# DaehwanKimLab/centrifuge

Measured on NVIDIA H100. Metric: reads/sec (100 bp SE classification), higher is better.
Workload: dtype u64

## Files before the change

### centrifuge_b200/csrc/cfb200.cu

```cuda
#include "../../include/cfb200.h"
#include "cf_index.h"
#include "cf_kernels.cuh"
#include <cub/cub.cuh>

#include <algorithm>
#include <atomic>
#include <mutex>
#include <thread>
#include <fcntl.h>
#include <unistd.h>
#include <cstdarg>
#include <cstdio>
#include <cstring>
#include <set>
#include <string>
#include <vector>

using namespace cfb;

enum { M_DONE = 0, M_FTAB = 1, M_LF = 2, M_NEED = 3, M_FTABK = 4, M_TASK = 5 };

struct SearchArgs {
	IndexView v; Params p; BatchView b;
	HitRec* hits; uint32_t* nhits; uint32_t cap;
// ... 31 lines not shown
	const int mate = (int)(rem >> 1), strand = (int)(rem & 1);
	const uint32_t len = mate ? a.b.len[1][unit] : a.b.len[0][unit];
	uint64_t w = 0; uint32_t n = 0;
	if(k * 32 < len) {
		const uint64_t off = mate ? a.b.off[1][unit] : a.b.off[0][unit];
		const uint32_t cnt = min(32u, len - k * 32);
		const uint64_t lo = strand ? off + k * 32 : off + (len - k * 32 - cnt);
		#pragma unroll
		for(uint32_t g = 0; g < 32; g += 4) {
			if(g < cnt) {
				const uint32_t keep = cnt - g >= 4 ? 0xffffffffu : ((1u << (8 * (cnt - g))) - 1u);
				const uint32_t v = load4(a.b.bases, lo + g) & keep;
				const uint32_t nb = __vcmpne4(v & 0xFCFCFCFCu, 0u) & 0x01010101u;
				uint32_t b2 = v & 0x03030303u;
				if(strand) b2 ^= 0x03030303u & keep;
				b2 &= ~(nb * 3u);
				w |= (uint64_t)squeeze4x2(b2) << (2 * g);
				n |= squeeze4x1(nb) << g;
			}
		}
		if(!strand) {
			uint64_t x = __brevll(w);
			x = ((x >> 1) & 0x5555555555555555ull) | ((x & 0x5555555555555555ull) << 1);
			w = x >> (2 * (32 - cnt)); n = __brev(n) >> (32 - cnt);
		}
	}
	a.pk[i] = w; a.nm[i] = n;
}

struct WarpPool { unsigned long long base = 0, end = 0, next = 0; bool ahead = false; };
__device__ __forceinline__ void pool_ahead(WarpPool& P, unsigned long long* ctr, unsigned chunk) {
	if(!P.ahead && P.end - P.base < 32) { if((threadIdx.x & 31) == 0) P.next = atomicAdd(ctr, (unsigned long long)chunk); P.ahead = true; }
}
__device__ __forceinline__ bool pool_take(WarpPool& P, bool want, unsigned long long* ctr, unsigned long long total, unsigned chunk, unsigned long long& out) {
	const unsigned need = __ballot_sync(0xffffffffu, want);
	if(!need) return false;
	const unsigned lane = threadIdx.x & 31;
	const unsigned cnt = __popc(need), r = __popc(need & ((1u << lane) - 1u));
	const unsigned long long avail = P.end - P.base;
	unsigned long long nb = 0;
	const bool refill = avail < cnt;
	if(refill) { if(lane == 0) nb = P.ahead ? P.next : atomicAdd(ctr, (unsigned long long)chunk); nb = __shfl_sync(0xffffffffu, nb, 0); P.ahead = false; }
	unsigned long long t, lim;
	if(r < avail) { t = P.base + r; lim = P.end; }
	else { t = nb + (r - avail); lim = nb + chunk < total ? nb + chunk : total; }
	if(refill) { P.base = nb + (cnt - avail); P.end = nb + chunk < total ? nb + chunk : total; if(P.base > P.end) P.base = P.end; }
	else P.base += cnt;
	out = t;
	return want && t < lim;
}

__device__ __forceinline__ uint64_t even_bits(uint64_t x) {
	x &= 0x5555555555555555ull;
	x = (x | (x >> 1)) & 0x3333333333333333ull;
	x = (x | (x >> 2)) & 0x0f0f0f0f0f0f0f0full;
	x = (x | (x >> 4)) & 0x00ff00ff00ff00ffull;
	x = (x | (x >> 8)) & 0x0000ffff0000ffffull;
	x = (x | (x >> 16)) & 0x00000000ffffffffull;
	return x;
}

__global__ void k_build_rank16(const uint64_t* sides, uint64_t num_sides, uint64_t zside, uint32_t zoffc, uint64_t* r16) {
	const uint64_t b = (uint64_t)blockIdx.x * blockDim.x + threadIdx.x;
	if(b > num_sides * 6) return;
	const bool sentinel = b == num_sides * 6;
	const uint64_t s = sentinel ? num_sides - 1 : b / 6; const uint32_t sub = sentinel ? 6u : (uint32_t)(b - s * 6);
	const uint64_t* sd = sides + s * 16;
	uint64_t occ[4] = {sd[12], sd[13], sd[14], sd[15]};
	for(uint32_t k = 0; k < sub * 2; k++) {
		const uint64_t w = sd[k];
		const uint64_t lo = w & 0x5555555555555555ull, hi = (w >> 1) & 0x5555555555555555ull;
		const uint32_t c1 = __popcll(lo & ~hi), c2 = __popcll(hi & ~lo), c3 = __popcll(hi & lo);
		occ[1] += c1; occ[2] += c2; occ[3] += c3; occ[0] += 32 - c1 - c2 - c3;
	}
	if(s == zside && zoffc < sub * 64) occ[0] -= 1;
	for(int c = 0; c < 4; c++) {
		uint64_t bits = 0;
		if(!sentinel) {
			bits = even_bits(match2(sd[sub * 2], c)) | (even_bits(match2(sd[sub * 2 + 1], c)) << 32);
			if(c == 0 && s == zside && zoffc >= sub * 64 && zoffc < sub * 64 + 64) bits &= ~(1ull << (zoffc - sub * 64));
		}
		r16[(b * 4 + c) * 2] = occ[c]; r16[(b * 4 + c) * 2 + 1] = bits;
	}
}
__global__ void k_mark_boundaries(const uint64_t* brow, uint32_t n, uint64_t* r16) {
	const uint32_t i = blockIdx.x * blockDim.x + threadIdx.x;
	if(i < n) atomicOr((unsigned long long*)&r16[(brow[i] >> 6) * 8], 1ull << 63);
}
__global__ void k_build_ftab2(IndexView v, uint64_t n, uint64_t* ftab2) {
	const uint64_t fi = (uint64_t)blockIdx.x * blockDim.x + threadIdx.x;
	if(fi >= n) return;
	ftab2[fi * 2] = ftab_hi(v, v.ftab[fi]); ftab2[fi * 2 + 1] = ftab_lo(v, v.ftab[fi + 1]);
}
static const uint32_t kListNoLong = 0x80000000u;
static const uint32_t kListRegen = 0x40000000u;
static const uint32_t kLongLen = 22;
__host__ __device__ __forceinline__ uint32_t nh_pack(uint32_t stored, uint32_t found, bool nolong) {
	return (stored & 0x7fffu) | ((found < 0x7fffu ? found : 0x7fffu) << 15) | (nolong ? kListNoLong : 0u);
}
__host__ __device__ __forceinline__ uint32_t nh_stored(uint32_t w) { return w & 0x7fffu; }
__host__ __device__ __forceinline__ uint32_t nh_found(uint32_t w) { return (w >> 15) & 0x7fffu; }

static const uint64_t kFtabkWide = 0xFFFFFFull;
__device__ __forceinline__ uint32_t ftabk_death(uint64_t y, uint32_t e) {
	if((y >> e) & 1ull) return 0;
	if(!(y & (0x1111111111111111ull << (e & 3u)))) return 1;
	if(!(y & (0x0001000100010001ull << (e & 15u)))) return 2;
	return 3;
}
__device__ __forceinline__ void lf4(const IndexView& v, const ulonglong2* r16, uint64_t top, uint64_t bot, uint64_t t[4], uint64_t b[4]) {
	const ulonglong2* pt = r16 + r16_entry(top, 0); const ulonglong2* pb = r16 + r16_entry(bot, 0);
	#pragma unroll
	for(int c = 0; c < 4; c++) {
		const ulonglong2 et = __ldg(pt + c); const ulonglong2 eb = (pb == pt) ? et : __ldg(pb + c);
		t[c] = r16_lf(v, top, c, et.x, et.y);
		b[c] = r16_lf(v, bot, c, eb.x, eb.y);
	}
}
__global__ void __launch_bounds__(128) k_build_ftabk(IndexView v, int K, uint64_t n, bool death, ulonglong2* out) {
	const uint64_t fk = (uint64_t)blockIdx.x * blockDim.x + threadIdx.x;
	if(fk >= n) return;
	const ulonglong2* r16 = reinterpret_cast<const ulonglong2*>(v.rank16);
	const int fc = v.ftab_chars;
	const uint64_t f10 = fk & ((1ull << (2 * fc)) - 1ull);
	uint64_t top = v.ftab2[f10 * 2], bot = v.ftab2[f10 * 2 + 1];
	for(int j = fc; j < K && bot > top; j++) {
		const int c = (int)((fk >> (2 * j)) & 3);
		const ulonglong2 tq = __ldg(r16 + r16_entry(top, c)), bq = __ldg(r16 + r16_entry(bot, c));
		top = r16_lf(v, top, c, tq.x, tq.y);
		bot = r16_lf(v, bot, c, bq.x, bq.y);
	}
	if(bot <= top) { out[fk] = make_ulonglong2(0ull, ~0ull); return; }
	uint64_t y = ~0ull;
	if(death) {
		uint8_t dv[64];
		uint64_t t1[4], b1[4]; lf4(v, r16, top, bot, t1, b1);
		for(int c0 = 0; c0 < 4; c0++) {
			if(b1[c0] <= t1[c0]) { for(int r = 0; r < 16; r++) dv[c0 | (r << 2)] = 1; continue; }
			uint64_t t2[4], b2[4]; lf4(v, r16, t1[c0], b1[c0], t2, b2);
			for(int c1 = 0; c1 < 4; c1++) {
				if(b2[c1] <= t2[c1]) { for(int c2 = 0; c2 < 4; c2++) dv[c0 | (c1 << 2) | (c2 << 4)] = 2; continue; }
				uint64_t t3[4], b3[4]; lf4(v, r16, t2[c1], b2[c1], t3, b3);
				for(int c2 = 0; c2 < 4; c2++) dv[c0 | (c1 << 2) | (c2 << 4)] = b3[c2] <= t3[c2] ? 3 : 0;
			}
		}
		y = 0;
		for(int e = 0; e < 64; e++) if(dv[e] == 0) y |= 1ull << e;
		for(uint32_t e = 0; e < 64; e++) if(ftabk_death(y, e) != dv[e]) { y = ~0ull; break; }
	}
	const uint64_t w = bot - top;
	out[fk] = make_ulonglong2(top | ((w < kFtabkWide ? w : kFtabkWide) << 40), y);
}

template <int RW> struct ReadRegs {
	uint64_t rw[RW]; uint32_t nw[RW];
	__device__ __forceinline__ uint64_t word(uint32_t k) const {
		uint64_t v = 0;
		#pragma unroll
		for(int q = 0; q < RW; q++) if((uint32_t)q == k) v = rw[q];
		return v;
	}
	__device__ __forceinline__ uint32_t nword(uint32_t k) const {
		uint32_t v = 0;
		#pragma unroll
		for(int q = 0; q < RW; q++) if((uint32_t)q == k) v = nw[q];
		return v;
	}
	__device__ __forceinline__ int base(uint32_t p) const {
		const uint32_t k = p >> 5, sh = p & 31;
		return ((nword(k) >> sh) & 1u) ? 4 : (int)((word(k) >> (2 * sh)) & 3);
	}
	__device__ __forceinline__ void window(uint32_t p, uint64_t& win, uint32_t& nwin) const {
		const uint32_t k = p >> 5, sh = p & 31;
		win = shr64(word(k), 2 * sh) | shl64(word(k + 1), 64 - 2 * sh);
		nwin = (uint32_t)(((uint64_t)nword(k) | ((uint64_t)nword(k + 1) << 32)) >> sh);
	}
};

__device__ __forceinline__ void ld_if(ulonglong2& v, const void* p) {
	asm volatile("{\n\t.reg .pred p;\n\tsetp.ne.u64 p, %2, 0;\n\t@p ld.global.nc.v2.u64 {%0, %1}, [%2];\n\t}" : "+l"(v.x), "+l"(v.y) : "l"(p));
}
__device__ __forceinline__ void ld_if(uint64_t& v, const uint64_t* p, bool on) {
	asm volatile("{\n\t.reg .pred p;\n\tsetp.ne.u32 p, %2, 0;\n\t@p ld.global.nc.u64 %0, [%1];\n\t}" : "+l"(v) : "l"(p), "r"((uint32_t)on));
}
__device__ __forceinline__ void ld_if(uint32_t& v, const uint32_t* p, bool on) {
	asm volatile("{\n\t.reg .pred p;\n\tsetp.ne.u32 p, %2, 0;\n\t@p ld.global.nc.u32 %0, [%1];\n\t}" : "+r"(v) : "l"(p), "r"((uint32_t)on));
}
__device__ __forceinline__ void ld_if(uint32_t& v, const uint8_t* p, bool on) {
	asm volatile("{\n\t.reg .pred p;\n\tsetp.ne.u32 p, %2, 0;\n\t@p ld.global.nc.u8 %0, [%1];\n\t}" : "+r"(v) : "l"(p), "r"((uint32_t)on));
}

template <bool REQS, int RW>
__global__ void __launch_bounds__(kSearchThreads, !REQS && RW <= 5 ? 8 : 1) k_search_t(const SearchArgs a) {
	const ulonglong2* r16 = reinterpret_cast<const ulonglong2*>(a.v.rank16);
	const ulonglong2* ftab2 = reinterpret_cast<const ulonglong2*>(a.v.ftab2);
	const ulonglong2* ftabk = reinterpret_cast<const ulonglong2*>(a.v.ftabk);
	const uint32_t fk = a.v.ftabk ? (uint32_t)a.v.ftabk_chars : 0u;
	const uint32_t fc = (uint32_t)a.v.ftab_chars;
	const unsigned long long* w8 = reinterpret_cast<const unsigned long long*>(a.v.walk8);
	const uint32_t fd = (fk == 0 || a.p.min_hitlen < (uint32_t)a.v.ftabd_chars) ? 0u : (uint32_t)a.v.ftabd_chars;
	const uint32_t msh = a.b.n_mates == 2 ? 2u : 1u;
	ReadRegs<RW> rd;
	#pragma unroll
	for(int k = 0; k < RW; k++) { rd.rw[k] = 0; rd.nw[k] = 0; }
	uint64_t top = 0, bot = 0, fi = 0;
	uint32_t rlen = 0, tid = 0, cur = 0, dep = 0, offset = 0, nh = 0, nt = 0, slow_until = 0, fail_at = 0xffffffffu;
	bool nolong = true;
	int mode = M_NEED;
	unsigned long long q_r16 = 0, q_f2 = 0, q_fk = 0, q_w8 = 0;
	unsigned long long q_w1 = 0, q_w24 = 0, q_w5 = 0, j_row = 0, j_row_ok = 0, j_rng = 0, j_rng_ok = 0, j_w5_ok = 0;
	unsigned long long s_trips = 0, s_lreq = 0, s_cons = 0, s_rest = 0, s_task = 0, s_head = 0, s_wait = 0, s_tail = 0;
	uint32_t paths = 0; long long t_top = 0, t_issue = 0, t_data = 0;
	WarpPool pool;
	bool more = true;

	for(;;) {
		if(REQS) { paths = 0; t_top = clock64(); }
		{
			const bool want = mode == M_NEED;
			if(more) {
				unsigned long long t = 0;
				const bool got = pool_take(pool, want, a.task_ctr64, (unsigned long long)a.ntasks, a.chunk, t);
				if(want) {
					if(got) { tid = (uint32_t)t; mode = M_TASK; if(REQS) paths |= 1u << 17; }
					else mode = M_DONE;
				}
				if(__any_sync(0xffffffffu, want && !got)) more = false;
				else pool_ahead(pool, a.task_ctr64, a.chunk);
			} else if(want) mode = M_DONE;
		}
		if(!__any_sync(0xffffffffu, mode != M_DONE)) break;
		int c = 4;
		const bool lf = mode == M_LF, task = mode == M_TASK;
		bool range = false, jump = false, known_fail = false;
		const void* p0 = nullptr; const void* p1 = nullptr; uint32_t sub = 0;
		if(mode == M_FTAB) { p0 = ftab2 + fi; if(REQS) q_f2++; }
		else if(mode == M_FTABK) { p0 = ftabk + (fi & ((1ull << (2 * fk)) - 1ull)); if(REQS) q_fk++; }
		else if(lf) {
			c = rd.base(dep);
			if(c <= 3) {
				range = (bot - top) != 1;
				const uint64_t width = bot - top;
				if(dep == fail_at && !range) known_fail = true;
				else if(w8 && dep >= slow_until && rlen - dep >= 8 && bot <= a.v.walk8_rows) {
					jump = true; p0 = w8 + (top & ~1ull); sub = (uint32_t)(top & 1);
					if(range) { const uint64_t last = bot - 1; sub |= (uint32_t)(last & 1) << 1; if((last & ~1ull) != (top & ~1ull)) p1 = w8 + (last & ~1ull); }
					if(REQS) { q_w8 += p1 ? 2 : 1; if(range) j_rng++; else j_row++; }
				} else {
					p0 = r16 + r16_entry(top, c);
					if(range && (bot >> 6) != (top >> 6)) p1 = r16 + r16_entry(bot, c);
					if(REQS) { const uint32_t n = p1 ? 2 : 1; q_r16 += n; if(width == 1) q_w1 += n; else if(width <= 4) q_w24 += n; else q_w5 += n; }
				}
			}
		}
		const uint32_t unit = tid >> msh, mate = (tid >> 1) & (msh - 1u);
		const uint64_t* tpk = a.pk + (size_t)tid * a.W; const uint32_t* tnm = a.nm + (size_t)tid * a.W;
		uint32_t fl = 3;
		if(REQS) { if(p0) s_lreq++; t_issue = clock64(); }
		const bool two = p1 != nullptr;
		ulonglong2 e = make_ulonglong2(0, 0), e2 = make_ulonglong2(0, 0);
		ld_if(e, p0);
		ld_if(e2, p1);
		ld_if(rlen, (mate ? a.b.len[1] : a.b.len[0]) + unit, task);
		ld_if(fl, a.b.flags + unit, task && a.b.flags != nullptr);
		#pragma unroll
		for(int k = 0; k < RW; k++) { ld_if(rd.rw[k], tpk + k, task && (uint32_t)k < a.W); ld_if(rd.nw[k], tnm + k, task && (uint32_t)k < a.W); }
		if(REQS) {
			if(__any_sync(0xffffffffu, (e.x ^ e2.y ^ rd.rw[RW - 1] ^ rd.nw[RW - 1] ^ rlen ^ fl) == 0x9e3779b97f4a7c15ull)) s_task += 1ull << 40;
			t_data = clock64();
		}
		const ulonglong2 tq = e, bq = two ? e2 : e;
		bool ended = false, stop = false, fresh = false;
		uint64_t h_top = kOff, h_bot = kOff; uint32_t hl = 0;
		if(task) {
			if(REQS) paths |= 1u;
			#pragma unroll
			for(int k = 0; k < RW; k++) if((uint32_t)k >= a.W) { rd.rw[k] = 0; rd.nw[k] = 0; }
			nh = 0; nt = 0;
			if(!((fl >> mate) & 1) || rlen == 0) { a.nhits[tid] = 0; mode = M_NEED; }
			else { cur = 0; slow_until = 0; fail_at = 0xffffffffu; nolong = true; fresh = true; }
		} else if(mode == M_FTABK) {
			if(REQS) paths |= 2u;
			const uint32_t ext = (uint32_t)(fi >> (2 * fk));
			const uint32_t dv = ext ? ftabk_death(e.y, ext & 63u) : 0u;
			const uint64_t width = e.x >> 40;
			if(dv) {
				hl = fk + dv - 1u; h_top = h_bot = kUnk; cur += hl; ended = true;
			} else if(width != 0 && width != kFtabkWide) {
				top = e.x & kRowMask; bot = top + width; dep = cur + fk;
				if(dep < rlen) mode = M_LF; else stop = true;
			} else { fi &= (1ull << (2 * fc)) - 1ull; mode = M_FTAB; }
		} else if(mode == M_FTAB) {
			if(REQS) paths |= 4u;
			top = e.x; bot = e.y;
			dep = cur + fc;
			if(bot <= top) { hl = dep - offset; cur = dep; ended = true; }
			else if(dep < rlen) mode = M_LF;
			else stop = true;
		} else if(jump) {
			if(REQS) paths |= 8u;
			uint64_t win; uint32_t nwin; rd.window(dep, win, nwin);
			const uint64_t w = (sub & 1u) ? e.y : e.x;
			const uint64_t wl = range ? ((sub & 2u) ? bq.y : bq.x) : w;
			const uint32_t st = walk8_steps(w, win, nwin), sb = range ? walk8_steps(wl, win, nwin) : st;
			if((st & sb) == 8u) {
				if(REQS) { if(range) j_rng_ok++; else j_row_ok++; if(bot - top >= 5) j_w5_ok++; }
				top = w & kWalkRowMask; bot = (wl & kWalkRowMask) + 1; dep += 8;
				stop = dep >= rlen;
			} else {
				slow_until = dep + walk8_retry(st, sb);
				if(!range) fail_at = dep + st;
			}
		} else if(lf) {
			if(REQS) paths |= 16u;
			bool fail = c > 3 || known_fail;
			uint64_t t = 0, b = 0;
			if(!fail) {
				t = r16_lf(a.v, top, c, tq.x, tq.y);
				if(range) b = r16_lf(a.v, bot, c, bq.x, bq.y);
				else {
					if(!((tq.y >> (top & 63)) & 1ull)) fail = true;
					b = t + 1;
				}
				if(b <= t) fail = true;
			}
			if(fail) stop = true;
			else { top = t; bot = b; dep++; stop = dep >= rlen; }
		}
		if(stop) { h_top = top; h_bot = bot; hl = dep - offset; cur = dep; ended = true; }
		#pragma unroll 1
		while(ended || fresh) {
			if(ended) {
				if(REQS) paths |= 1u << 16;
				if(a.keep_short || hl >= kLongLen) {
					if(nh < a.cap) { HitRec* h = a.hits + (size_t)tid * a.cap + nh; h->top = h_top; h->bot = h_bot; h->bwoff = offset; h->len = hl; }
					else atomicExch(a.overflow, 1u);
					nh++;
				}
				nt++;
				if(hl >= a.p.min_hitlen) nolong = false;
				ended = false;
				bool done = cur >= rlen;
				if(!done) { if(hl > a.p.increment) cur += 1; if(cur + a.p.min_hitlen >= rlen) done = true; }
				if(done) { a.nhits[tid] = nh_pack(nh, nt, nolong); mode = M_NEED; break; }
			}
			if(REQS) paths |= 1u << 18;
			fresh = false;
			offset = cur; h_top = h_bot = kOff;
			if(rlen - cur < fc) { hl = rlen - cur; cur = rlen; ended = true; continue; }
			uint64_t win; uint32_t nwin; rd.window(cur, win, nwin);
			const uint32_t nbits = nwin & ((1u << fc) - 1u);
			if(nbits) { hl = (uint32_t)__ffs(nbits); cur += hl; ended = true; continue; }
			if(fk && rlen - cur >= fk && !(nwin & ((1u << fk) - 1u))) {
				fi = win & ((1ull << (2 * fk)) - 1ull);
				if(fd && rlen - cur >= fd && !(nwin & ((1u << fd) - 1u))) fi |= (64ull | ((win >> (2 * fk)) & 63ull)) << (2 * fk);
				mode = M_FTABK;
			} else {
				fi = win & ((1ull << (2 * fc)) - 1ull);
				mode = M_FTAB;
			}
		}
		if(REQS) {
			const uint32_t all = __reduce_or_sync(0xffffffffu, paths);
			s_trips++; s_cons += __popc(all & 0xffffu); s_rest += __popc(all >> 16); if(all & (1u << 17)) s_task++;
			const long long t_end = clock64(); s_head += t_issue - t_top; s_wait += t_data - t_issue; s_tail += t_end - t_data;
		}
	}
	if(REQS && a.ctr) {
		atomicAdd(&a.ctr->req_rank16, q_r16); atomicAdd(&a.ctr->req_ftab2, q_f2); atomicAdd(&a.ctr->req_ftabk, q_fk); atomicAdd(&a.ctr->req_walk8, q_w8);
		atomicAdd(&a.ctr->r16_w1, q_w1); atomicAdd(&a.ctr->r16_w2_4, q_w24); atomicAdd(&a.ctr->r16_w5, q_w5);
		atomicAdd(&a.ctr->w8_try_row, j_row); atomicAdd(&a.ctr->w8_ok_row, j_row_ok); atomicAdd(&a.ctr->w8_try_range, j_rng); atomicAdd(&a.ctr->w8_ok_range, j_rng_ok); atomicAdd(&a.ctr->w8_ok_w5, j_w5_ok);
		atomicAdd(&a.ctr->it_lane_req, s_lreq);
		if((threadIdx.x & 31) == 0) {
			atomicAdd(&a.ctr->it_warp, s_trips); atomicAdd(&a.ctr->it_consumers, s_cons); atomicAdd(&a.ctr->it_restarts, s_rest); atomicAdd(&a.ctr->it_task, s_task & ((1ull << 40) - 1ull));
			atomicAdd(&a.ctr->clk_head, s_head); atomicAdd(&a.ctr->clk_wait, s_wait); atomicAdd(&a.ctr->clk_tail, s_tail);
		}
	}
}

struct UnitArgs {
	IndexView v; Params p; BatchView b;
	HitRec* hits; uint32_t* nhits; uint32_t cap;
	uint32_t* nrows;
	uint64_t* row_off;
	unsigned long long* row_total;
	uint64_t* rows; uint32_t* ids; uint64_t rows_cap;
	Entry* entries; TaxCnt* tcs; OutRec* recs_sparse; uint32_t* nout;
	unsigned int* overflow;
	Counters* ctr;
	HitRec* regen; uint32_t* regen_n; unsigned long long* regen_ctr; uint64_t regen_slots; uint32_t full_cap; uint32_t keep_short;
};

__device__ uint32_t search_strand_dev(const IndexView& v, const Params& p, const uint8_t* fw, uint32_t len, int strand, HitRec* hits, uint32_t cap) {
	const ulonglong2* r16 = reinterpret_cast<const ulonglong2*>(v.rank16);
	const ulonglong2* ftab2 = reinterpret_cast<const ulonglong2*>(v.ftab2);
	const ulonglong2* ftabk = reinterpret_cast<const ulonglong2*>(v.ftabk);
	const uint32_t fc = (uint32_t)v.ftab_chars, fk = v.ftabk ? (uint32_t)v.ftabk_chars : 0u;
	auto base = [&](uint32_t d) -> int { return seq_at(fw, len, strand, len - 1 - d); };
	uint32_t cur = 0, n = 0;
	if(len == 0) return 0;
	for(;;) {
		HitRec h; h.bwoff = cur; uint32_t new_cur; bool done = false;
		const uint32_t offset = cur;
		if(len - cur < fc) { h.top = h.bot = kOff; h.len = len - offset; new_cur = len; done = true; }
		else {
			uint32_t firstn = 0xffffffffu; uint64_t fi = 0;
			const uint32_t span = (fk && len - cur >= fk) ? fk : fc;
			for(uint32_t i = 0; i < span; i++) { const int c = base(cur + i); if(c > 3) { firstn = i; break; } fi |= (uint64_t)c << (2 * i); }
			if(firstn < fc) { new_cur = cur + firstn + 1; h.top = h.bot = kOff; h.len = new_cur - offset; done = new_cur >= len; }
			else {
				uint64_t top = 0, bot = 0; uint32_t dep = 0; bool have = false;
				if(span == fk && fk > fc && firstn == 0xffffffffu) {
					const uint64_t x = __ldg(&ftabk[fi].x), width = x >> 40;
					if(width != 0 && width != kFtabkWide) { top = x & kRowMask; bot = top + width; dep = cur + fk; have = true; }
				}
				if(!have) { const ulonglong2 e = __ldg(ftab2 + (fi & ((1ull << (2 * fc)) - 1ull))); top = e.x; bot = e.y; dep = cur + fc; }
				if(bot <= top) { h.top = h.bot = kOff; h.len = dep - offset; new_cur = dep; done = dep >= len; }
				else {
					uint32_t slow_until = 0;
					while(dep < len) {
						const int c = base(dep);
						if(c > 3) break;
						if(v.walk8 && bot <= v.walk8_rows && len - dep >= 8 && dep >= slow_until) {
							uint64_t win = 0; uint32_t nwin = 0;
							for(uint32_t j = 0; j < 8; j++) { const int b = base(dep + j); if(b > 3) nwin |= 1u << j; else win |= (uint64_t)b << (2 * j); }
							const uint64_t et = __ldg(v.walk8 + top), eb = bot - top == 1 ? et : __ldg(v.walk8 + bot - 1);
							const uint32_t st = walk8_steps(et, win, nwin), sb = walk8_steps(eb, win, nwin);
							if((st & sb) == 8u) { top = et & kWalkRowMask; bot = (eb & kWalkRowMask) + 1; dep += 8; continue; }
							slow_until = dep + walk8_retry(st, sb);
						}
// ... 834 lines not shown
	const uint8_t* src_bases = b->bases;
	if(!pinned(b->bases)) { CK(s.h_bases.ensure(b->n_bases)); memcpy(s.h_bases.p, b->bases, b->n_bases); src_bases = s.h_bases.p; }
	CK(cudaMemcpyAsync(s.d_bases.p, src_bases, b->n_bases, cudaMemcpyHostToDevice, s.st));
	CK(s.h_off.ensure(n * nm)); CK(s.h_len.ensure(n * nm)); CK(s.h_flags.ensure(n));
	for(int m = 0; m < nm; m++) {
		const uint64_t* so = b->off[m]; const uint32_t* sl = b->len[m];
		if(!pinned(so)) { memcpy(s.h_off.p + m * n, so, n * 8); so = s.h_off.p + m * n; }
		if(!pinned(sl)) { memcpy(s.h_len.p + m * n, sl, n * 4); sl = s.h_len.p + m * n; }
		CK(cudaMemcpyAsync(s.d_off.p + m * n, so, n * 8, cudaMemcpyHostToDevice, s.st));
		CK(cudaMemcpyAsync(s.d_len.p + m * n, sl, n * 4, cudaMemcpyHostToDevice, s.st));
	}
	if(b->flags && pinned(b->flags)) CK(cudaMemcpyAsync(s.d_flags.p, b->flags, n, cudaMemcpyHostToDevice, s.st));
	else { if(b->flags) memcpy(s.h_flags.p, b->flags, n); else memset(s.h_flags.p, 3, n); CK(cudaMemcpyAsync(s.d_flags.p, s.h_flags.p, n, cudaMemcpyHostToDevice, s.st)); }
	s.bv.bases = s.d_bases.p; s.bv.flags = s.d_flags.p; s.bv.n_units = (uint32_t)n; s.bv.n_mates = nm;
	for(int m = 0; m < 2; m++) { s.bv.off[m] = m < nm ? s.d_off.p + m * n : nullptr; s.bv.len[m] = m < nm ? s.d_len.p + m * n : nullptr; }
	s.n_units = n; s.n_bases = b->n_bases; s.maxlen = maxlen;
	(void)c;
	return CFB_OK;
}

__global__ void __launch_bounds__(256) k_wlen(const uint32_t* len, uint64_t n, uint32_t* wlen) {
	const uint64_t i = (uint64_t)blockIdx.x * blockDim.x + threadIdx.x;
	if(i < n) wlen[i] = (len[i] + 31u) >> 5;
}
__global__ void __launch_bounds__(256) k_unpack(const uint64_t* __restrict__ words, const uint64_t* __restrict__ woff, uint64_t wbase, const uint32_t* __restrict__ len,
                                                uint64_t n, uint32_t W, uint8_t* bases, uint64_t* off) {
	const uint64_t t = (uint64_t)blockIdx.x * blockDim.x + threadIdx.x;
	if(t >= n * W) return;
	const uint64_t i = t / W; const uint32_t k = (uint32_t)(t - i * W);
	const uint64_t w0 = wbase + woff[i];
	if(k == 0) off[i] = w0 * 32;
	if(k * 32 >= len[i]) return;
	const uint64_t w = __ldg(words + w0 + k);
	uint32_t o[8];
	#pragma unroll
	for(int q = 0; q < 8; q++) {
		const uint32_t b = (uint32_t)(w >> (8 * q)) & 0xffu;
		o[q] = (b & 3u) | ((b & 0xcu) << 6) | ((b & 0x30u) << 12) | ((b & 0xc0u) << 18);
	}
	uint4* dst = reinterpret_cast<uint4*>(bases + (w0 + k) * 32);
	dst[0] = make_uint4(o[0], o[1], o[2], o[3]); dst[1] = make_uint4(o[4], o[5], o[6], o[7]);
}
__global__ void __launch_bounds__(256) k_set_n(const uint64_t* npos, uint64_t n, uint8_t* bases, uint64_t limit) {
	const uint64_t i = (uint64_t)blockIdx.x * blockDim.x + threadIdx.x;
	if(i < n) { const uint64_t p = npos[i]; if(p < limit) bases[p] = 4; }
}

static int stage_batch_packed(cfb_ctx* c, Slot& s, const cfb_batch_packed* b) {
	if(!b || b->n_mates < 1 || b->n_mates > 2 || !b->words || !b->len[0] || (b->n_mates == 2 && !b->len[1]) || (b->n_n && !b->n_pos))
		return fail(CFB_EINVAL, "malformed cfb_batch_packed");
	if(b->n_units >= (1ull << 30)) return fail(CFB_EINVAL, "batch too large (n_units must be < 2^30)");
	const uint64_t n = b->n_units; const int nm = b->n_mates;
	uint32_t maxlen = 0; uint64_t need_words = 0, mate_words[2] = {0, 0};
	for(int m = 0; m < nm; m++) {
		const uint32_t* L = b->len[m]; uint32_t mx = 0; uint64_t w = 0;
		for(uint64_t i = 0; i < n; i++) { const uint32_t l = L[i]; mx = l > mx ? l : mx; w += (l + 31u) >> 5; }
		maxlen = std::max(maxlen, mx); mate_words[m] = w; need_words += w;
	}
	if(need_words != b->n_words) return fail(CFB_EINVAL, "cfb_batch_packed: n_words is %llu, the lengths need %llu", (unsigned long long)b->n_words, (unsigned long long)need_words);
	if(maxlen > 60000) return fail(CFB_EINVAL, "read longer than 60000 bases");
	const uint64_t scan_blocks = (n + kScanBlock * kScanPer - 1) / (kScanBlock * kScanPer);
	CK(s.d_bases.ensure(b->n_words * 32 + 64)); CK(s.d_off.ensure(n * nm + 1)); CK(s.d_len.ensure(n * nm)); CK(s.d_flags.ensure(n));
	CK(s.d_words.ensure(b->n_words + 1)); CK(s.d_npos.ensure(b->n_n + 1)); CK(s.d_wlen.ensure(n + 1)); CK(s.d_woff.ensure(n + 2)); CK(s.bsum.ensure(scan_blocks + 1));
	auto pinned = [](const void* p) -> bool {
		cudaPointerAttributes at;
		if(cudaPointerGetAttributes(&at, p) != cudaSuccess) { cudaGetLastError(); return false; }
		return at.type == cudaMemoryTypeHost;
	};
	const uint64_t* src_words = b->words;
	if(!pinned(b->words)) { CK(s.h_words.ensure(b->n_words)); memcpy(s.h_words.p, b->words, b->n_words * 8); src_words = s.h_words.p; }
	CK(cudaMemcpyAsync(s.d_words.p, src_words, b->n_words * 8, cudaMemcpyHostToDevice, s.st));
	CK(s.h_len.ensure(n * nm)); CK(s.h_flags.ensure(n));
	for(int m = 0; m < nm; m++) {
		const uint32_t* sl = b->len[m];
		if(!pinned(sl)) { memcpy(s.h_len.p + m * n, sl, n * 4); sl = s.h_len.p + m * n; }
		CK(cudaMemcpyAsync(s.d_len.p + m * n, sl, n * 4, cudaMemcpyHostToDevice, s.st));
	}
	if(b->n_n) {
		const uint64_t* sp = b->n_pos;
		if(!pinned(sp)) { CK(s.h_off.ensure(b->n_n)); memcpy(s.h_off.p, sp, b->n_n * 8); sp = s.h_off.p; }
		CK(cudaMemcpyAsync(s.d_npos.p, sp, b->n_n * 8, cudaMemcpyHostToDevice, s.st));
	}
	if(b->flags && pinned(b->flags)) CK(cudaMemcpyAsync(s.d_flags.p, b->flags, n, cudaMemcpyHostToDevice, s.st));
	else { if(b->flags) memcpy(s.h_flags.p, b->flags, n); else memset(s.h_flags.p, 3, n); CK(cudaMemcpyAsync(s.d_flags.p, s.h_flags.p, n, cudaMemcpyHostToDevice, s.st)); }
	const uint32_t W = (maxlen + 31) / 32;
	uint64_t wbase = 0;
	CK(cudaMemsetAsync(s.scal.p + 5, 0, 8, s.st));
	for(int m = 0; m < nm && n; m++) {
		k_wlen<<<(unsigned)((n + 255) / 256), 256, 0, s.st>>>(s.d_len.p + m * n, n, s.d_wlen.p);
		k_scan_sums<<<(unsigned)scan_blocks, kScanBlock, 0, s.st>>>(s.d_wlen.p, n, s.bsum.p);
		k_scan_top<<<1, 1024, 0, s.st>>>(s.bsum.p, scan_blocks, (uint64_t*)(s.scal.p + 5));
		k_scan_apply<<<(unsigned)scan_blocks, kScanBlock, 0, s.st>>>(s.d_wlen.p, n, s.bsum.p, (const uint64_t*)(s.scal.p + 5), s.d_woff.p);
		if(W) k_unpack<<<(unsigned)((n * W + 255) / 256), 256, 0, s.st>>>(s.d_words.p, s.d_woff.p, wbase, s.d_len.p + m * n, n, W, s.d_bases.p, s.d_off.p + m * n);
		c->launches += 5;
		wbase += mate_words[m];
	}
	if(b->n_n) { k_set_n<<<(unsigned)((b->n_n + 255) / 256), 256, 0, s.st>>>(s.d_npos.p, b->n_n, s.d_bases.p, b->n_words * 32); c->launches++; }
	CK(cudaGetLastError());
	s.bv.bases = s.d_bases.p; s.bv.flags = s.d_flags.p; s.bv.n_units = (uint32_t)n; s.bv.n_mates = nm;
	for(int m = 0; m < 2; m++) { s.bv.off[m] = m < nm ? s.d_off.p + m * n : nullptr; s.bv.len[m] = m < nm ? s.d_len.p + m * n : nullptr; }
	s.n_units = n; s.n_bases = b->n_words * 32; s.maxlen = maxlen;
	return CFB_OK;
}

static int enqueue_kernels(cfb_ctx* c, Slot& s, int stage, bool time_it) {
	const uint64_t n = s.n_units; const int nm = s.bv.n_mates;
	const uint64_t ntasks = n * nm * 2;
	const uint32_t ublocks = (uint32_t)((n + 127) / 128);
	const uint64_t scan_blocks = (n + kScanBlock * kScanPer - 1) / (kScanBlock * kScanPer);
	if(n == 0) return CFB_OK;
	const SearchKernel search = search_kernel(s.maxlen, c->count);
	const bool keep_short = search == k_search_long<true> || search == k_search_long<false> || c->prm.min_hitlen < kLongLen || c->keep_short;
	if(stage == 0) {
		if(s.cap == 0) {
			s.full_cap = s.maxlen / 4 + 8;
			s.cap = keep_short ? s.full_cap : s.maxlen / kLongLen + 2;
		}
		CK(s.hits.ensure(ntasks * s.cap)); CK(s.nhits.ensure(ntasks));
		if(!keep_short) {
			s.regen_slots = std::max<uint64_t>(s.regen_slots, c->regen_slots0 ? c->regen_slots0 : std::max<uint64_t>(ntasks / 32, 1024));
			CK(s.regen.ensure(s.regen_slots * s.full_cap)); CK(s.regen_n.ensure(s.regen_slots));
			CK(cudaMemsetAsync(s.scal.p + 6, 0, sizeof(unsigned long long), s.st));
		}
		const uint32_t W = (s.maxlen + 31) / 32 + 1;
		CK(s.pk.ensure(ntasks * W + 2)); CK(s.nm.ensure(ntasks * W + 2)); CK(s.nrows.ensure(n)); CK(s.row_off.ensure(n + 1));
		CK(s.bsum.ensure(scan_blocks + 1)); CK(s.nout.ensure(n + 1)); CK(s.out_off.ensure(n + 1)); CK(s.rec_off32.ensure(n + 1));
		s.rows_cap = std::max<uint64_t>(s.rows_cap, c->rows_cap0 ? c->rows_cap0 : std::max<uint64_t>(n * 12, 4096));
	}
	CK(s.rows.ensure(s.rows_cap)); CK(s.ids.ensure(s.rows_cap)); CK(s.entries.ensure(s.rows_cap)); CK(s.tcs.ensure(s.rows_cap)); CK(s.sparse.ensure(s.rows_cap));
	s.dense_cap = s.rows_cap; CK(s.dense.ensure(s.dense_cap));
	CK(cudaMemsetAsync(s.scal.p, 0, 4 * sizeof(unsigned long long), s.st));
	if(time_it) CK(cudaEventRecord(s.ev[0], s.st));
	Counters* ctr = c->count ? c->d_ctr : nullptr;
	if(c->count && stage == 0) CK(cudaMemsetAsync(c->d_ctr, 0, sizeof(Counters), s.st));
	else if(c->count) {
		const size_t sc0 = offsetof(Counters, sc_units);
		CK(cudaMemsetAsync(reinterpret_cast<char*>(c->d_ctr) + sc0, 0, sizeof(Counters) - sc0, s.st));
	}
	UnitArgs ua; ua.v = c->view; ua.p = c->prm; ua.b = s.bv; ua.hits = s.hits.p; ua.nhits = s.nhits.p; ua.cap = s.cap;
	ua.nrows = s.nrows.p; ua.row_off = s.row_off.p; ua.row_total = s.scal.p + 3; ua.rows = s.rows.p; ua.ids = s.ids.p; ua.rows_cap = s.rows_cap;
	ua.entries = s.entries.p; ua.tcs = s.tcs.p; ua.recs_sparse = s.sparse.p; ua.nout = s.nout.p;
	ua.overflow = (unsigned int*)(s.scal.p + 2); ua.ctr = ctr;
	ua.regen = s.regen.p; ua.regen_n = s.regen_n.p; ua.regen_ctr = s.scal.p + 6; ua.regen_slots = s.regen_slots; ua.full_cap = s.full_cap; ua.keep_short = keep_short ? 1u : 0u;
	if(stage == 0) {
		SearchArgs sa; sa.v = c->view; sa.p = c->prm; sa.b = s.bv; sa.hits = s.hits.p; sa.nhits = s.nhits.p; sa.cap = s.cap;
		const uint32_t W = (s.maxlen + 31) / 32 + 1;
		sa.pk = s.pk.p; sa.nm = s.nm.p; sa.W = W; sa.keep_short = keep_short ? 1u : 0u;
		{ PackArgs pa; pa.b = s.bv; pa.pk = s.pk.p; pa.nm = s.nm.p; pa.W = W;
		  k_pack<<<(unsigned)((ntasks * W + 127) / 128), 128, 0, s.st>>>(pa); c->launches++; }
		sa.task_ctr64 = s.scal.p + 0; sa.ntasks = (uint32_t)ntasks; sa.overflow = (unsigned int*)(s.scal.p + 2); sa.ctr = ctr;
		int occ = 1;
		CK(cudaOccupancyMaxActiveBlocksPerMultiprocessor(&occ, search, kSearchThreads, 0));
		const uint64_t resident = (uint64_t)c->ix->sm_count * (uint64_t)std::max(occ, 1);
		const uint64_t warps = resident * (kSearchThreads / 32);
		sa.chunk = (uint32_t)std::min<uint64_t>(std::max<uint64_t>(ntasks / (warps * 4), 32), 256);
		const int blocks = (int)std::min<uint64_t>(resident, (ntasks + kSearchThreads - 1) / kSearchThreads);
		search<<<blocks, kSearchThreads, 0, s.st>>>(sa);
		c->launches++;
		if(time_it) CK(cudaEventRecord(s.ev[1], s.st));
		k_prep<8, false><<<ublocks, 128, 0, s.st>>>(ua); c->launches++;
	} else {
		if(time_it) CK(cudaEventRecord(s.ev[1], s.st));
		k_prep<8, true><<<ublocks, 128, 0, s.st>>>(ua); c->launches++;
	}
	if(time_it) CK(cudaEventRecord(s.ev[2], s.st));
	ResolveArgs ra; ra.v = c->view; ra.rows = s.rows.p; ra.ids = s.ids.p; ra.ids16 = nullptr; ra.total = (const uint64_t*)(s.scal.p + 3); ra.rows_cap = s.rows_cap;
	ra.task_ctr = s.scal.p + 1; ra.chunk = 64; ra.ctr = ctr;
	if((c->view.rtab16 || c->view.rtab32) && c->count != 1) k_lookup<<<c->ix->sm_count * 8, 256, 0, s.st>>>(ra);
	else if(c->count) k_resolve_c<true, false><<<c->resolve_blocks, kSearchThreads, 0, s.st>>>(ra);
	else k_resolve_c<false, false><<<c->resolve_blocks, kSearchThreads, 0, s.st>>>(ra);
	c->launches++;
	if(time_it) CK(cudaEventRecord(s.ev[3], s.st));
	if(ctr) k_score<12, true><<<ublocks, kScoreThreads, 0, s.st>>>(ua);
	else k_score<12, false><<<ublocks, kScoreThreads, 0, s.st>>>(ua);
	size_t scan_bytes = 0;
	CK(cub::DeviceScan::ExclusiveScan(nullptr, scan_bytes, s.nout.p, s.out_off.p, cub::Sum(), (uint64_t)0, (int)(n + 1), s.st));
	CK(s.scan_tmp.ensure(scan_bytes));
	CK(cudaMemsetAsync(s.nout.p + n, 0, sizeof(uint32_t), s.st));
	CK(cub::DeviceScan::ExclusiveScan(s.scan_tmp.p, scan_bytes, s.nout.p, s.out_off.p, cub::Sum(), (uint64_t)0, (int)(n + 1), s.st));
	CK(cudaMemcpyAsync(s.scal.p + 4, s.out_off.p + n, sizeof(uint64_t), cudaMemcpyDeviceToDevice, s.st));
	k_compact<<<(unsigned)((n + 1 + 127) / 128), 128, 0, s.st>>>((uint32_t)n, s.row_off.p, s.out_off.p, s.sparse.p, s.dense.p, s.rec_off32.p, s.dense_cap, (unsigned int*)(s.scal.p + 2));
	c->launches += 4;
	s.folded = false;
	if(c->fold_records && !s.is_text) {
		const uint32_t nsp = c->cnt.n;
		CK(s.cnt.ensure(3ull * nsp)); CK(cudaMemsetAsync(s.cnt.p, 0, 3ull * nsp * 8, s.st));
		FoldArgs fa; fa.sp_taxid = c->cnt.d_taxid.p; fa.n_sp = nsp; fa.rec_off = s.rec_off32.p; fa.recs = s.dense.p; fa.n_units = (uint32_t)n; fa.n_mates = nm;
		fa.khits = c->prm.khits; fa.len[0] = s.bv.len[0]; fa.len[1] = s.bv.len[1]; fa.flags = s.bv.flags; fa.sp = s.cnt.p;
		k_fold_counts<<<ublocks, 128, 0, s.st>>>(fa); c->launches++;
		s.folded = true;
	}
	if(time_it) CK(cudaEventRecord(s.ev[4], s.st));
	s.d2h_recs = 0;
	if(s.want_host) {
		const uint64_t guess = std::min<uint64_t>(s.dense_cap, (uint64_t)((double)n * c->rec_ratio * 1.05) + 4096);
		CK(s.h_recs.ensure(guess + 1)); CK(s.h_rec_off.ensure(n + 1));
		CK(cudaMemcpyAsync(s.h_rec_off.p, s.rec_off32.p, (n + 1) * 4, cudaMemcpyDeviceToHost, s.st));
		CK(cudaMemcpyAsync(s.h_recs.p, s.dense.p, guess * sizeof(OutRec), cudaMemcpyDeviceToHost, s.st));
		s.d2h_recs = guess;
	}
	CK(cudaMemcpyAsync(s.h_scal.p, s.scal.p, 8 * sizeof(unsigned long long), cudaMemcpyDeviceToHost, s.st));
	CK(cudaGetLastError());
	return CFB_OK;
}

static int finish_batch(cfb_ctx* c, Slot& s, bool time_it, bool to_host, cfb_result* out) {
	if(s.n_units == 0) { if(out) { out->n_units = 0; out->n_recs = 0; out->rec_off = nullptr; out->recs = nullptr; } return CFB_OK; }
	for(int attempt = 0; attempt < 8; attempt++) {
		CK(cudaStreamSynchronize(s.st));
		const unsigned ovf = (unsigned)(s.h_scal.p[2] & 0xffffffffu);
		const uint64_t total_rows = s.h_scal.p[3];
		if(ovf == 4) {
			s.regen_slots = s.h_scal.p[6] + s.h_scal.p[6] / 4 + 1024; s.reran = true;
			int rc = enqueue_kernels(c, s, 0, time_it); if(rc) return rc;
			continue;
		}
		if(ovf == 1) {
			s.cap = s.maxlen + 2; s.full_cap = s.maxlen + 2; s.reran = true;
			int rc = enqueue_kernels(c, s, 0, time_it); if(rc) return rc;
			continue;
		}
		if(total_rows > s.rows_cap) {
			s.rows_cap = total_rows + total_rows / 4 + 1024; s.reran = true;
			int rc = enqueue_kernels(c, s, 1, time_it); if(rc) return rc;
			continue;
		}
		if(ovf != 0) return fail(CFB_ECUDA, "internal capacity error %u", ovf);
		break;
	}
	const uint64_t nrec = s.h_scal.p[4];
	c->regen_lists += s.h_scal.p[6]; c->regen_tasks += (uint64_t)s.n_units * (uint64_t)s.bv.n_mates * 2;
	if(s.folded) {
		const uint32_t n3 = 3 * c->cnt.n;
		k_cnt_commit<<<(n3 + 255) / 256, 256, 0, s.st>>>(s.cnt.p, c->cnt.total.p, n3); c->launches++;
		CK(cudaEventRecord(s.ev[5], s.st)); s.commit_pending = true;
		s.folded = false; c->cnt.reduced = false;
	}
	if(to_host) {
		if(s.n_units) c->rec_ratio = std::max(c->rec_ratio * 0.98, (double)nrec / (double)s.n_units);
		if(!s.want_host || nrec > s.d2h_recs) {
			const uint64_t have = s.want_host ? s.d2h_recs : 0;
			if(nrec + 1 > s.h_recs.cap) {
				CK(s.h_recs.ensure(nrec + 1));
				if(nrec) CK(cudaMemcpyAsync(s.h_recs.p, s.dense.p, nrec * sizeof(OutRec), cudaMemcpyDeviceToHost, s.st));
			} else if(nrec > have) CK(cudaMemcpyAsync(s.h_recs.p + have, s.dense.p + have, (nrec - have) * sizeof(OutRec), cudaMemcpyDeviceToHost, s.st));
			if(!s.want_host) { CK(s.h_rec_off.ensure(s.n_units + 1)); CK(cudaMemcpyAsync(s.h_rec_off.p, s.rec_off32.p, (s.n_units + 1) * 4, cudaMemcpyDeviceToHost, s.st)); }
			CK(cudaStreamSynchronize(s.st));
		}
	}
	if(out) { out->n_units = s.n_units; out->n_recs = nrec; out->rec_off = s.h_rec_off.p; out->recs = reinterpret_cast<const cfb_rec*>(s.h_recs.p); }
	return CFB_OK;
}

extern "C" int cfb_classify_submit(cfb_ctx* c, int slot, const cfb_batch* b) {
	if(!c || slot < 0 || slot >= kSlots - 1) return fail(CFB_EINVAL, "bad ctx/slot");
	CK(cudaSetDevice(c->ix->device));
	Slot& s = c->slots[slot];
	if(s.pending) return fail(CFB_EINVAL, "slot %d still has an un-waited batch", slot);
	int rc = stage_batch(c, s, b); if(rc) return rc;
	s.cap = 0; s.want_host = true; s.is_text = false;
	rc = enqueue_kernels(c, s, 0, false); if(rc) return rc;
	s.pending = true;
	return CFB_OK;
}
extern "C" int cfb_classify_submit_packed(cfb_ctx* c, int slot, const cfb_batch_packed* b) {
	if(!c || slot < 0 || slot >= kSlots - 1) return fail(CFB_EINVAL, "bad ctx/slot");
	CK(cudaSetDevice(c->ix->device));
	Slot& s = c->slots[slot];
	if(s.pending) return fail(CFB_EINVAL, "slot %d still has an un-waited batch", slot);
	int rc = stage_batch_packed(c, s, b); if(rc) return rc;
	s.cap = 0; s.want_host = true; s.is_text = false;
	rc = enqueue_kernels(c, s, 0, false); if(rc) return rc;
	s.pending = true;
	return CFB_OK;
}
extern "C" int cfb_pack_batch(const cfb_batch* in, uint64_t* words, uint64_t words_cap, uint64_t* n_pos, uint64_t npos_cap, uint64_t* n_words, uint64_t* n_n) {
	if(!in || !n_words || !n_n || in->n_mates < 1 || in->n_mates > 2) return fail(CFB_EINVAL, "cfb_pack_batch: bad argument");
	uint64_t w = 0, nn = 0; bool fits = true;
	for(int m = 0; m < in->n_mates; m++) for(uint64_t i = 0; i < in->n_units; i++) {
		const uint8_t* p = in->bases + in->off[m][i]; const uint32_t len = in->len[m][i];
		for(uint32_t k = 0; k < len; k += 32) {
			uint64_t v = 0; const uint32_t cnt = std::min<uint32_t>(32, len - k);
			for(uint32_t j = 0; j < cnt; j++) {
				const uint8_t c = p[k + j];
				if(c > 3) { if(n_pos && nn < npos_cap) n_pos[nn] = (w << 5) | j; else fits = false; nn++; }
				else v |= (uint64_t)c << (2 * j);
			}
			if(words && w < words_cap) words[w] = v; else fits = false;
			w++;
		}
	}
	*n_words = w; *n_n = nn;
	return fits ? CFB_OK : fail(CFB_EINVAL, "cfb_pack_batch: buffers too small (%llu words, %llu N positions needed)", (unsigned long long)w, (unsigned long long)nn);
}
extern "C" int cfb_classify_wait(cfb_ctx* c, int slot, cfb_result* out) {
	if(!c || slot < 0 || slot >= kSlots - 1 || !out) return fail(CFB_EINVAL, "bad ctx/slot");
	CK(cudaSetDevice(c->ix->device));
	Slot& s = c->slots[slot];
	if(!s.pending) return fail(CFB_EINVAL, "slot %d has no submitted batch", slot);
	s.pending = false;
	return finish_batch(c, s, false, true, out);
}
extern "C" int cfb_classify_batch(cfb_ctx* c, const cfb_batch* b, cfb_result* out) {
	int rc = cfb_classify_submit(c, 0, b); if(rc) return rc;
	return cfb_classify_wait(c, 0, out);
}

extern "C" int cfb_batch_upload(cfb_ctx* c, const cfb_batch* b, cfb_dbatch** out) {
// ... 85 lines not shown
```

Before: 302.0 million.

## Stage packed read words in shared memory via cp.async instead of registers

Per-thread packed read words and N-masks now live in a shared-memory array indexed [word][thread] and are filled with predicated cp.async copies, replacing register arrays that were selected with unrolled compare chains. This is meant to cut register pressure so larger RW variants can also request 8 blocks per SM, and to turn dynamic word indexing into a direct shared load. The work-pool chunk size is also fixed at 32 instead of being derived from the number of resident warps. The cost is extra shared-memory traffic on every base and window lookup, shared-memory usage that may limit occupancy for large RW, and a wait_all on each new task.

Result: faster. 308.2 million (median of 6 runs) (+2.1%).

```diff
diff --git a/centrifuge_b200/csrc/cfb200.cu b/centrifuge_b200/csrc/cfb200.cu
--- a/centrifuge_b200/csrc/cfb200.cu
+++ b/centrifuge_b200/csrc/cfb200.cu
@@ -207,20 +207,10 @@
 	out[fk] = make_ulonglong2(top | ((w < kFtabkWide ? w : kFtabkWide) << 40), y);
 }
 
-template <int RW> struct ReadRegs {
-	uint64_t rw[RW]; uint32_t nw[RW];
-	__device__ __forceinline__ uint64_t word(uint32_t k) const {
-		uint64_t v = 0;
-		#pragma unroll
-		for(int q = 0; q < RW; q++) if((uint32_t)q == k) v = rw[q];
-		return v;
-	}
-	__device__ __forceinline__ uint32_t nword(uint32_t k) const {
-		uint32_t v = 0;
-		#pragma unroll
-		for(int q = 0; q < RW; q++) if((uint32_t)q == k) v = nw[q];
-		return v;
-	}
+template <int RW> struct ReadSmem {
+	uint64_t* w; uint32_t* n;
+	__device__ __forceinline__ uint64_t word(uint32_t k) const { return w[k * kSearchThreads]; }
+	__device__ __forceinline__ uint32_t nword(uint32_t k) const { return n[k * kSearchThreads]; }
 	__device__ __forceinline__ int base(uint32_t p) const {
 		const uint32_t k = p >> 5, sh = p & 31;
 		return ((nword(k) >> sh) & 1u) ? 4 : (int)((word(k) >> (2 * sh)) & 3);
@@ -232,6 +222,14 @@
 	}
 };
 
+template <int BYTES>
+__device__ __forceinline__ void cp_async_if(void* dst, const void* src, bool on, bool fill) {
+	const uint32_t d = (uint32_t)__cvta_generic_to_shared(dst);
+	asm volatile("{\n\t.reg .pred p;\n\tsetp.ne.u32 p, %3, 0;\n\t@p cp.async.ca.shared.global [%0], [%1], %4, %2;\n\t}"
+	             :: "r"(d), "l"(src), "r"(fill ? (uint32_t)BYTES : 0u), "r"((uint32_t)on), "n"(BYTES) : "memory");
+}
+__device__ __forceinline__ void cp_async_wait_all() { asm volatile("cp.async.wait_all;" ::: "memory"); }
+
 __device__ __forceinline__ void ld_if(ulonglong2& v, const void* p) {
 	asm volatile("{\n\t.reg .pred p;\n\tsetp.ne.u64 p, %2, 0;\n\t@p ld.global.nc.v2.u64 {%0, %1}, [%2];\n\t}" : "+l"(v.x), "+l"(v.y) : "l"(p));
 }
@@ -246,7 +244,7 @@
 }
 
 template <bool REQS, int RW>
-__global__ void __launch_bounds__(kSearchThreads, !REQS && RW <= 5 ? 8 : 1) k_search_t(const SearchArgs a) {
+__global__ void __launch_bounds__(kSearchThreads, REQS ? 1 : 8) k_search_t(const SearchArgs a) {
 	const ulonglong2* r16 = reinterpret_cast<const ulonglong2*>(a.v.rank16);
 	const ulonglong2* ftab2 = reinterpret_cast<const ulonglong2*>(a.v.ftab2);
 	const ulonglong2* ftabk = reinterpret_cast<const ulonglong2*>(a.v.ftabk);
@@ -255,9 +253,11 @@
 	const unsigned long long* w8 = reinterpret_cast<const unsigned long long*>(a.v.walk8);
 	const uint32_t fd = (fk == 0 || a.p.min_hitlen < (uint32_t)a.v.ftabd_chars) ? 0u : (uint32_t)a.v.ftabd_chars;
 	const uint32_t msh = a.b.n_mates == 2 ? 2u : 1u;
-	ReadRegs<RW> rd;
+	__shared__ uint64_t s_pk[RW + 1][kSearchThreads];
+	__shared__ uint32_t s_nm[RW + 1][kSearchThreads];
+	const ReadSmem<RW> rd = { &s_pk[0][threadIdx.x], &s_nm[0][threadIdx.x] };
 	#pragma unroll
-	for(int k = 0; k < RW; k++) { rd.rw[k] = 0; rd.nw[k] = 0; }
+	for(int k = 0; k <= RW; k++) { s_pk[k][threadIdx.x] = 0; s_nm[k][threadIdx.x] = 0; }
 	uint64_t top = 0, bot = 0, fi = 0;
 	uint32_t rlen = 0, tid = 0, cur = 0, dep = 0, offset = 0, nh = 0, nt = 0, slow_until = 0, fail_at = 0xffffffffu;
 	bool nolong = true;
@@ -319,9 +319,14 @@
 		ld_if(rlen, (mate ? a.b.len[1] : a.b.len[0]) + unit, task);
 		ld_if(fl, a.b.flags + unit, task && a.b.flags != nullptr);
 		#pragma unroll
-		for(int k = 0; k < RW; k++) { ld_if(rd.rw[k], tpk + k, task && (uint32_t)k < a.W); ld_if(rd.nw[k], tnm + k, task && (uint32_t)k < a.W); }
+		for(int k = 0; k < RW; k++) {
+			const bool in = (uint32_t)k < a.W;
+			cp_async_if<8>(&s_pk[k][threadIdx.x], in ? tpk + k : tpk, task, in);
+			cp_async_if<4>(&s_nm[k][threadIdx.x], in ? tnm + k : tnm, task, in);
+		}
 		if(REQS) {
-			if(__any_sync(0xffffffffu, (e.x ^ e2.y ^ rd.rw[RW - 1] ^ rd.nw[RW - 1] ^ rlen ^ fl) == 0x9e3779b97f4a7c15ull)) s_task += 1ull << 40;
+			cp_async_wait_all();
+			if(__any_sync(0xffffffffu, (e.x ^ e2.y ^ rd.word(RW - 1) ^ rd.nword(RW - 1) ^ rlen ^ fl) == 0x9e3779b97f4a7c15ull)) s_task += 1ull << 40;
 			t_data = clock64();
 		}
 		const ulonglong2 tq = e, bq = two ? e2 : e;
@@ -329,8 +334,7 @@
 		uint64_t h_top = kOff, h_bot = kOff; uint32_t hl = 0;
 		if(task) {
 			if(REQS) paths |= 1u;
-			#pragma unroll
-			for(int k = 0; k < RW; k++) if((uint32_t)k >= a.W) { rd.rw[k] = 0; rd.nw[k] = 0; }
+			cp_async_wait_all();
 			nh = 0; nt = 0;
 			if(!((fl >> mate) & 1) || rlen == 0) { a.nhits[tid] = 0; mode = M_NEED; }
 			else { cur = 0; slow_until = 0; fail_at = 0xffffffffu; nolong = true; fresh = true; }
@@ -1471,8 +1475,7 @@
 		int occ = 1;
 		CK(cudaOccupancyMaxActiveBlocksPerMultiprocessor(&occ, search, kSearchThreads, 0));
 		const uint64_t resident = (uint64_t)c->ix->sm_count * (uint64_t)std::max(occ, 1);
-		const uint64_t warps = resident * (kSearchThreads / 32);
-		sa.chunk = (uint32_t)std::min<uint64_t>(std::max<uint64_t>(ntasks / (warps * 4), 32), 256);
+		sa.chunk = 32;
 		const int blocks = (int)std::min<uint64_t>(resident, (ntasks + kSearchThreads - 1) / kSearchThreads);
 		search<<<blocks, kSearchThreads, 0, s.st>>>(sa);
 		c->launches++;
```
